# Atarilab/iterative_learning_NMPC

Measured on AMD Instinct MI355X. Metric: MPC solves/sec (horizon-50 centroidal, batch), higher is better.
Workload: dtype f32; 1 GPU; configs[1]: batch=1024/GPU centroidal quadruped NMPC nx=12 nu=12 N=50 fp32, 1 SQP x 6 IPM Riccati sweeps per solve, warm-start shift + solve per step; global_batch=1024, horizon=50, parallelism=dp1 (independent problems; no collective)

## Files before the change

iterative_learning_nmpc_amd/csrc/nmpc_models.hpp:

```cpp
#pragma once
#include "nmpc_tile.hpp"

#pragma clang fp contract(off)

namespace nmpc {

struct ModelParams {
    float dt, mass, ixx, iyy, izz, gz, mu, umax;
    float p_gain, hipx, hipy, lhip, l1, l2, res0, res1;
};

struct DoubleIntegrator {
    static constexpr int ID = 0, NX = 4, NU = 2, NP = 0, NG = 4;

    __device__ static void step(const ModelParams& mp, const float (&x)[NX], const float (&u)[NU],
                                const float*, float (&xn)[NX]) {
        const float dt = mp.dt, h2 = 0.5f * dt * dt;
        xn[0] = x[0] + dt * x[2] + h2 * u[0];
        xn[1] = x[1] + dt * x[3] + h2 * u[1];
        xn[2] = x[2] + dt * u[0];
        xn[3] = x[3] + dt * u[1];
    }
    template <class EA, class EB>
    __device__ static void linearize(const ModelParams& mp, const float (&x)[NX], const float (&u)[NU],
                                     const float* p, float (&xn)[NX], EA&& emitA, EB&& emitB) {
        step(mp, x, u, p, xn);
        const float dt = mp.dt, h2 = 0.5f * dt * dt;
        { float c[NX] = {1.f, 0.f, 0.f, 0.f}; emitA(0, c); }
        { float c[NX] = {0.f, 1.f, 0.f, 0.f}; emitA(1, c); }
        { float c[NX] = {dt, 0.f, 1.f, 0.f}; emitA(2, c); }
        { float c[NX] = {0.f, dt, 0.f, 1.f}; emitA(3, c); }
        { float c[NX] = {h2, 0.f, dt, 0.f}; emitB(0, c); }
        { float c[NX] = {0.f, h2, 0.f, dt}; emitB(1, c); }
    }
    __device__ static float G(const ModelParams&, int j, int c) {
        return (c == (j >> 1)) ? ((j & 1) ? -1.f : 1.f) : 0.f;
    }
    __device__ static float h(const ModelParams& mp, int) { return mp.umax; }
    __device__ static unsigned active_mask(const ModelParams& mp, const float*) {
        return mp.umax > 0.f ? 0xFu : 0u;
    }
    __device__ static void gdot(const ModelParams&, const float (&v)[NU], float (&o)[NG]) {
#pragma clang fp contract(off)
        o[0] = v[0]; o[1] = -v[0]; o[2] = v[1]; o[3] = -v[1];
    }
    static constexpr int N_STATIC_MASKS = 1;
    __host__ __device__ static constexpr unsigned static_mask(int) { return 0x3u; }
    __host__ __device__ static constexpr int static_index(unsigned mask) { return mask == 0x3u ? 0 : -1; }
    __host__ __device__ static constexpr int common_variant(int i) { return i == 0 ? 0 : -1; }
    __host__ __device__ static constexpr unsigned barrier_steps(unsigned) { return 0xFu; }
    __device__ static unsigned input_mask(const ModelParams&, const float*) { return 0x3u; }
};

struct Centroidal {
    static constexpr int ID = 1, NX = 12, NU = 12, NP = 16, NG = 16;

    struct Trig { float cz, sz, cy, sy, cx, sx; };

    __device__ static void rot(const Trig& t, float (&R)[9]) {
        R[0] = t.cz * t.cy; R[1] = t.cz * t.sy * t.sx - t.sz * t.cx; R[2] = t.cz * t.sy * t.cx + t.sz * t.sx;
        R[3] = t.sz * t.cy; R[4] = t.sz * t.sy * t.sx + t.cz * t.cx; R[5] = t.sz * t.sy * t.cx - t.cz * t.sx;
        R[6] = -t.sy;       R[7] = t.cy * t.sx;                       R[8] = t.cy * t.cx;
    }
    __device__ static void tmul(const float (&M)[9], const float (&v)[3], float (&o)[3]) {
        o[0] = M[0] * v[0] + M[3] * v[1] + M[6] * v[2];
        o[1] = M[1] * v[0] + M[4] * v[1] + M[7] * v[2];
        o[2] = M[2] * v[0] + M[5] * v[1] + M[8] * v[2];
    }

    struct Core {
        Trig t; float R[9]; float F[3]; float tau[3]; float w[3]; float vn[3]; float wn[3]; float T[9];
    };
    __device__ static void core(const ModelParams& mp, const float (&x)[NX], const float (&u)[NU],
                                const float* p, Core& k) {
        sincosf(x[3], &k.t.sz, &k.t.cz);
        sincosf(x[4], &k.t.sy, &k.t.cy);
        sincosf(x[5], &k.t.sx, &k.t.cx);
        rot(k.t, k.R);
        k.w[0] = x[11]; k.w[1] = x[10]; k.w[2] = x[9];
        k.F[0] = k.F[1] = k.F[2] = 0.f;
        k.tau[0] = k.tau[1] = k.tau[2] = 0.f;
#pragma unroll
        for (int i = 0; i < 4; ++i) {
            const float c = p[i];
// ... 152 lines not shown
        const int d = c - 3 * f;
        return (d == (jj >> 1)) ? ((jj & 1) ? -1.f : 1.f) : (d == 2 ? -mp.mu : 0.f);
    }
    __device__ static float h(const ModelParams&, int) { return 0.f; }
    __device__ static unsigned active_mask(const ModelParams&, const float* p) {
        unsigned m = 0;
#pragma unroll
        for (int f = 0; f < 4; ++f) m |= (p[f] > 0.5f) ? (0x1111u << f) : 0u;
        return m;
    }
    __device__ static unsigned input_mask(const ModelParams&, const float* p) {
        unsigned m = 0;
#pragma unroll
        for (int f = 0; f < 4; ++f) m |= (p[f] > 0.5f) ? (0x7u << (3 * f)) : 0u;
        return m;
    }
    static constexpr int N_STATIC_MASKS = 16;
    __host__ __device__ static constexpr unsigned static_mask(int i) {
        unsigned m = 0;
        for (int f = 0; f < 4; ++f) m |= ((i >> f) & 1) ? (0x7u << (3 * f)) : 0u;
        return m;
    }
    __host__ __device__ static constexpr int common_variant(int i) { return i == 0 ? 9 : i == 1 ? 6 : i == 2 ? 15 : i == 3 ? 0 : -1; }
    __host__ __device__ static constexpr unsigned barrier_steps(unsigned mask) {
        unsigned m = 0;
        for (int f = 0; f < 4; ++f) m |= ((mask >> (3 * f)) & 1u) << f;
        return m;
    }
    __host__ __device__ static constexpr int static_index(unsigned mask) {
        int i = 0;
        for (int f = 0; f < 4; ++f) i |= ((mask >> (3 * f)) & 1u) << f;
        return static_mask(i) == mask ? i : -1;
    }
    __device__ static void gdot(const ModelParams& mp, const float (&v)[NU], float (&o)[NG]) {
#pragma clang fp contract(off)
#pragma unroll
        for (int f = 0; f < 4; ++f) {
            o[row_of(f, 0)] = __builtin_fmaf(-mp.mu, v[3 * f + 2], v[3 * f]);
            o[row_of(f, 1)] = __builtin_fmaf(-mp.mu, v[3 * f + 2], -v[3 * f]);
            o[row_of(f, 2)] = __builtin_fmaf(-mp.mu, v[3 * f + 2], v[3 * f + 1]);
            o[row_of(f, 3)] = __builtin_fmaf(-mp.mu, v[3 * f + 2], -v[3 * f + 1]);
        }
    }
};

}

#pragma clang fp contract(fast)
```

iterative_learning_nmpc_amd/csrc/nmpc_solve.hip:

```cpp
#include <hip/hip_runtime.h>

#include <type_traits>

#include "../../include/nmpc.h"
#include "nmpc_models.hpp"
#include "nmpc_sweep.hpp"

namespace nmpc {

struct SolveArgs {
    ModelParams mp;
    float W[32];
    float rs_free[16];
    float We[16];
    float reg, reg_e;
    int N, B;
    int max_sqp, n_ipm, line_search, yref_per_stage;
    int it;
    int shift;
    float nlp_tol, mu0, sigma, s_min, gamma, tau_min, rho;
    const float* x0;
    const float* yref;
    const float* yref_e;
    const float* params;
// ... 112 lines not shown
        int o = 0;
        Xs = o;  o += round4(nX);
        Us = o;  o += round4(nU);
        dX = o;  o += round4(nX);
        dU = o;  o += round4(nU);
        dXp = o; o += round4(nX);
        dUp = o; o += round4(nU);
        sv = o;  o += round4(nG);
        lv = o;  o += round4(nG);
        o += 4;
        total = o;
    }
};

template <class M>
struct WsLayout {
    size_t At, Bt, Kt, Ct, q, r, c, act, umk, cost, flag, lean, stride;
    __host__ __device__ explicit WsLayout(int N) {
        size_t o = 0;
        At = o; o += (size_t)N * TileGeom<M>::A_FLOATS;
        Bt = o; o += (size_t)N * TileGeom<M>::B_FLOATS;
        Kt = o; o += (size_t)(N + 1) * TileGeom<M>::K_FLOATS;
        Ct = o; o += (size_t)(N + 1) * TileGeom<M>::C_FLOATS;
        q = o; o += round4((N + 1) * M::NX);
        r = o; o += round4(N * M::NU);
        c = o; o += round4(N * M::NG);
        act = o; o += round4(N);
        umk = o; o += round4(N);
        cost = o; o += round4(N + 1);
        flag = o; o += 4;
        lean = o; o += StageArrays<M>(N, true).total;
        stride = (o + 63) & ~(size_t)63;
    }
};
constexpr int N_LANE_STAGES = 4;
__host__ __device__ constexpr bool qp_linearizes_itself(bool lean, int N) { return lean && N < 64; }

#ifdef NMPC_STAMPS
#define STAMP_DECL unsigned long long st_t0 = __builtin_readcyclecounter(), st_acc[8] = {0, 0, 0, 0, 0, 0, 0, 0}; \
    StageStamps sst = {0, {0, 0, 0, 0, 0, 0, 0, 0}}
#define SST_PASS , sst
#define SST_TILES(i) SST(i)
#define STAMP(i) do { const unsigned long long st_t1 = __builtin_readcyclecounter(); st_acc[i] += st_t1 - st_t0; st_t0 = st_t1; } while (0)
#else
#define STAMP_DECL
#define STAMP(i)
#define SST_PASS
#define SST_TILES(i)
#endif

template <class M, bool LEAN>
struct Lds {
    int arr, qv, rv, gsq, gvt, act, umk, conv, dx0, total;
    __host__ __device__ explicit Lds(int N) {
        const int NS = (N + 1) | 1;
        int o = 0;
        arr = o; o += LEAN ? 0 : StageArrays<M>(N, false).total;
        qv = o;  o += (N + 1) * TS;
        rv = o;  o += N * TS;
        gsq = o; o += N * TS;
        gvt = o; o += N * TS;
        act = o; o += round4(NS);
        umk = o; o += round4(NS);
        conv = o; o += CONV_FLOATS;
        dx0 = o; o += LEAN ? TS : 0;
        total = o;
    }
};

constexpr int LIN_LDS_FLOATS = 64 * 16 + 2 * 64 * 2;
template <class M>
__device__ __forceinline__ void linearize_node(const SolveArgs& a, bool in_range, int b_in, int k_in, float* lds) {
#pragma clang fp contract(off)
    constexpr int NX = M::NX, NU = M::NU, NP = M::NP, NG = M::NG, NY = NX + NU;
    using G = TileGeom<M>;
    float* stage_col = lds;
    float** tile_of0 = reinterpret_cast<float**>(lds + 64 * 16);
    float** tile_of1 = tile_of0 + 64;
    float** tile_of[2] = {tile_of0, tile_of1};
    const int N = a.N;
    const int tid = threadIdx.x;
    const int b = b_in;
    const int k = in_range ? k_in : N;
    const WsLayout<M> wl(N);
    float* ws = a.ws + (size_t)b * wl.stride;
    const bool live = in_range && !(a.it > 0 && reinterpret_cast<const int*>(ws + wl.flag)[0]) && !skipped(a, b);
    const bool stage = live && k < N;
    const int ks = stage ? k : 0;
    const float* Xg = a.X + (size_t)b * (N + 1) * NX;
    const float* Ug = a.U + (size_t)b * N * NU;
    tile_of[0][tid] = stage ? ws + wl.At + (size_t)k * G::A_FLOATS : nullptr;
    tile_of[1][tid] = stage ? ws + wl.Bt + (size_t)k * G::B_FLOATS : nullptr;
    float x[NX];
#pragma unroll
    for (int i = 0; i < NX; ++i) x[i] = Xg[(size_t)shifted_node(live ? k : 0, a.shift, N) * NX + i];
    if (live && k == N) {
// ... 125 lines not shown
}

#pragma clang fp contract(off)
#ifndef NMPC_RES_WAVES
#define NMPC_RES_WAVES 1
#endif
template <class M, bool LEAN, bool BF16B, bool ALLV>
__global__ __launch_bounds__(64) __attribute__((amdgpu_waves_per_eu(LEAN ? 2 : NMPC_RES_WAVES, LEAN ? 2 : NMPC_RES_WAVES)))
void nmpc_qp_kernel(const SolveArgs a) {
    constexpr int NX = M::NX, NU = M::NU, NP = M::NP, NG = M::NG, NY = NX + NU;
    using G = TileGeom<M>;
    extern __shared__ __attribute__((aligned(16))) float smem[];
    const int b = blockIdx.x;
    if (b >= a.B) return;
    if (skipped(a, b)) return;
    const int lane = lane_id();
    const int q4 = lane >> 4, c = lane & 15;
    const int N = a.N;
    const WsLayout<M> wl(N);
    float* ws = a.ws + (size_t)b * wl.stride;
    int* flag = reinterpret_cast<int*>(ws + wl.flag);
    if (a.it > 0 && flag[0]) return;
    const Lds<M, LEAN> L(N);
    const StageArrays<M> SA_(N, LEAN);
    const int NS = SA_.NS;
    float* arr = LEAN ? ws + wl.lean : smem + L.arr;
    float* Xs = arr + SA_.Xs;   float* Us = arr + SA_.Us;
    float* dX = arr + SA_.dX;   float* dU = arr + SA_.dU;
    float* dXp = arr + SA_.dXp; float* dUp = arr + SA_.dUp;
    float* sv = arr + SA_.sv;   float* lv = arr + SA_.lv;
    float* idle_sink = arr + SA_.total - 4;
    float* qv = smem + L.qv;   float* rv = smem + L.rv;
    float* gsq = smem + L.gsq; float* gvt = smem + L.gvt;
    auto phase_sync = [&]() {
        if constexpr (LEAN) __threadfence_block();
        wave_sync();
    };
    unsigned* actm = reinterpret_cast<unsigned*>(smem + L.act);
    unsigned* umask = reinterpret_cast<unsigned*>(smem + L.umk);
    float* conv = smem + L.conv;
#define AT(arr, k, i) (arr)[LEAN ? (k) * TS + (i) : (i) * NS + (k)]
    auto ld_row = [&](const float* arr_, int k, auto& out) {
        constexpr int n = (int)(sizeof(out) / sizeof(float));
        if constexpr (LEAN) {
#pragma unroll
            for (int g = 0; g < (n + 3) / 4; ++g) {
                const f32x4 v = *reinterpret_cast<const f32x4*>(arr_ + k * TS + 4 * g);
#pragma unroll
                for (int r = 0; r < 4; ++r)
                    if (4 * g + r < n) out[4 * g + r] = v[r];
            }
        } else {
#pragma unroll
            for (int i = 0; i < n; ++i) out[i] = AT(arr_, k, i);
        }
    };
    auto st_row = [&](float* arr_, int k, const auto& in) {
        constexpr int n = (int)(sizeof(in) / sizeof(float));
        if constexpr (LEAN) {
#pragma unroll
            for (int g = 0; g < (n + 3) / 4; ++g) {
                f32x4 v;
#pragma unroll
                for (int r = 0; r < 4; ++r) v[r] = (4 * g + r < n) ? in[4 * g + r < n ? 4 * g + r : 0] : 0.0f;
                *reinterpret_cast<f32x4*>(arr_ + k * TS + 4 * g) = v;
            }
        } else {
#pragma unroll
            for (int i = 0; i < n; ++i) AT(arr_, k, i) = in[i];
        }
    };

    float* Xg = a.X + (size_t)b * (N + 1) * NX;
    float* Ug = a.U + (size_t)b * N * NU;
    const float* pg = a.params + (size_t)b * (N + 1) * NP;
    const float* yr = a.yref + (size_t)b * (a.yref_per_stage ? (size_t)N * NY : (size_t)NY);
    const float* yre = a.yref_e + (size_t)b * NX;
    const float* x0 = a.x0 + (size_t)b * NX;
    float* At = ws + wl.At;
    float* Bt = ws + wl.Bt;
    float* Kt = ws + wl.Kt;
    float* Ct = ws + wl.Ct;

    if constexpr (LEAN) {
        if (qp_linearizes_itself(LEAN, N)) {
            static_assert(LIN_LDS_FLOATS <= 4 * TS * 20, "scratch of the fused linearisation");
            linearize_node<M>(a, lane <= N, b, lane, smem + L.qv);
            __threadfence_block();
            wave_sync();
        }
    }
    for (int i = 4 * lane; i < L.conv; i += 256)
        *reinterpret_cast<f32x4*>(smem + i) = zero4();
    if constexpr (LEAN)
        for (int i = 4 * lane; i < SA_.total; i += 256) *reinterpret_cast<f32x4*>(arr + i) = zero4();
    phase_sync();
    constexpr int PRE = 13;
    auto fetch = [&](const float* src, int total, int base, float (&v)[PRE]) {
#pragma unroll
        for (int u = 0; u < PRE; ++u) {
            const int e = base + 64 * u + lane;
            v[u] = src[e < total ? e : 0];
// ... 44 lines not shown
        fetch(ws + wl.c, n_c, base, vc);
        drain(n_x, base, vx, put_x);
        drain(n_x, base, vq, put_q);
        drain(n_u, base, vu, put_u);
        drain(n_u, base, vr, put_r);
        drain(n_c, base, vc, put_c);
    }
    float* dx0s = smem + L.dx0;
    if constexpr (LEAN) {
        if (lane < NX) dx0s[lane] = x0[lane] - Xg[lane];
    }
    float cost_l = 0.0f, mu_l = 0.0f;
    int nact_l = 0;
    for (int k = lane; k <= N; k += 64) {
        cost_l += ws[wl.cost + k];
        if (k < N) {
            const unsigned am = reinterpret_cast<const unsigned*>(ws + wl.act)[k];
            actm[k] = am;
            const unsigned um = reinterpret_cast<const unsigned*>(ws + wl.umk)[k];
            const unsigned um_prev = reinterpret_cast<const unsigned*>(ws + wl.umk)[k > 0 ? k - 1 : 0];
            const unsigned wider = (k > 0 && (M::barrier_steps(um_prev) & ~M::barrier_steps(um)) != 0u) ? 1u : 0u;
            umask[k] = um | ((unsigned)(M::static_index(um) + 1) << 16) | (wider << 24);
            nact_l += __popc(am);
            mu_l += a.mu0 * (float)__popc(am);
        }
    }
    const int ic = index_of(c);
    const bool c_is_x = ic >= 0 && ic < NX, c_is_u = ic >= 0 && ic < NU;
    const float wq_c = c_is_x ? a.W[c_is_x ? ic : 0] + a.reg : 0.0f;
    const float wr_c = c_is_u ? a.W[NX + (c_is_u ? ic : 0)] + a.reg : 0.0f;
    const float we_c = c_is_x ? a.We[c_is_x ? ic : 0] + a.reg_e : 0.0f;
    SweepLane sl;
    sl.init(conv, lane, HS, a.rs_free);
    f32x4 Qc, Rc, Gc;
    bool qm[4], rm[4];
#pragma unroll
    for (int r = 0; r < 4; ++r) {
        const int row = 4 * q4 + r, ir = index_of(row);
        const bool r_is_x = ir >= 0 && ir < NX, r_is_u = ir >= 0 && ir < NU;
        Qc[r] = (row == c && r_is_x) ? wq_c : 0.0f;
        Rc[r] = (row == c && r_is_u) ? wr_c : 0.0f;
        qm[r] = (c == HS && r_is_x) || (row == HS && c_is_x);
        rm[r] = (c == HS && r_is_u);
        Gc[r] = (row < NG && c_is_u) ? M::G(a.mp, row < NG ? row : 0, c_is_u ? ic : 0) : 0.0f;
    }
    const bool is_hx_col = (c == HS);
    phase_sync();

    int status = NMPC_STATUS_MAXITER;
    bool finished = false;
    STAMP_DECL;
    float cost = 0.0f, stepn = 0.0f, alpha = 1.0f;
    const bool rows_in_regs = LEAN && N < 64;
    const int kx_s = lane <= N ? lane : 0, ku_s = lane < N ? lane : 0;
    float xr[LEAN ? NX : 1], ur[LEAN ? NU : 1];
    {
        cost = wave_sum(cost_l);
        const int n_act = (int)(wave_sum((float)nact_l) + 0.5f);
        STAMP(0);
        const bool use_ipm = (a.n_ipm > 0) && (n_act > 0);
        const int n_sweeps = use_ipm ? a.n_ipm : 1;
        bool qp_ok = true;
        float mu_sum = wave_sum(mu_l);
        const bool one_stage_per_lane = N <= 64;
        auto blend = [&](float ap) {
            batched<10>(SA_.nX, lane, [&](int i) { const float d = dX[i]; return __builtin_fmaf(ap, dXp[i] - d, d); },
                        [&](int i, float v) { dX[i] = v; });
            batched<10>(SA_.nU, lane, [&](int i) { const float d = dU[i]; return __builtin_fmaf(ap, dUp[i] - d, d); },
                        [&](int i, float v) { dU[i] = v; });
        };
        for (int ii = 0; ii < n_sweeps; ++ii) {
            float tau = 0.0f;
            if (use_ipm) {
                tau = fmaxf(a.sigma * mu_sum / (float)n_act, a.tau_min);
                if (ii == 0 || !one_stage_per_lane)
                for (int k = lane; k < N; k += 64) {
                    const unsigned am = actm[k];
                    float uk[NU], gk[NG], sk[NG], lk[NG];
                    ld_row(Us, k, uk);
                    ld_row(sv, k, sk);
                    ld_row(lv, k, lk);
                    M::gdot(a.mp, uk, gk);
#pragma unroll
                    for (int j = 0; j < NG; ++j) {
                        const bool on = (am >> j) & 1u;
                        const float s = sk[j], l = lk[j], cj = gk[j] - M::h(a.mp, j);
                        const float is = fast_rcp(s);
                        const float D = l * is;
                        const float rs = __builtin_amdgcn_rsqf(D);
                        gsq[k * TS + j] = on ? D * rs : 0.0f;
                        gvt[k * TS + j] = on ? __builtin_fmaf(D, cj, __builtin_fmaf(tau, is, l)) * rs : 0.0f;
                    }
                }
                phase_sync();
            }
            STAMP(1);
            f32x4 P;
            {
                const float qc = c_is_x ? qv[N * TS + c] : 0.0f;
#pragma unroll
                for (int r = 0; r < 4; ++r) {
                    const int row = 4 * q4 + r, ir = index_of(row);
                    const bool r_is_x = ir >= 0 && ir < NX;
                    float v = 0.0f;
                    if (row == c && r_is_x) v = we_c;
                    if (c == HS && r_is_x) v = qv[N * TS + row];
                    if (row == HS && c_is_x) v = qc;
                    P[r] = v;
                }
            }
            auto sweep = [&](auto ipm_tag) {
                constexpr bool IPM = decltype(ipm_tag)::value;
                struct NextCost {
                    f32x4 Gs, Vt, Tb, Qn, Sn, Rn;
                    const float *qrow, *rrow, *sqrow, *vtrow;
                    const float* qcol;
                    const bool *qm, *rm;
                    f32x4 Qc, Rc, Gc;
                    bool hx_col;
                    f32x4 q4v, r4v, sq4, vt4;
                    float qcv;
                    __device__ __forceinline__ void fetch() {
                        q4v = *reinterpret_cast<const f32x4*>(qrow);
                        r4v = *reinterpret_cast<const f32x4*>(rrow);
                        qcv = *qcol;
                        if constexpr (IPM) {
                            sq4 = *reinterpret_cast<const f32x4*>(sqrow);
                            vt4 = *reinterpret_cast<const f32x4*>(vtrow);
                        }
                    }
                    __device__ __forceinline__ void build() {
                        Rn = Rc;
#pragma unroll
                        for (int r = 0; r < 4; ++r) {
                            Qn[r] = Qc[r] + (qm[r] ? (hx_col ? q4v[r] : qcv) : 0.0f);
                            Sn[r] = rm[r] ? r4v[r] : 0.0f;
                        }
                        if constexpr (IPM) {
#pragma unroll
                            for (int r = 0; r < 4; ++r) {
                                Gs[r] = Gc[r] * sq4[r];
                                Vt[r] = hx_col ? vt4[r] : Gs[r];
                            }
                            Tb = zero4();
                        }
                    }
                    __device__ __forceinline__ void mfma(int i) {
                        if constexpr (IPM && !BF16B) Tb = __builtin_amdgcn_mfma_f32_16x16x4f32(Gs[i], Vt[i], Tb, 0, 0, 0);
                        if constexpr (IPM && BF16B) { if (i == 0) Tb = xty_bf16(Gs, Vt); }
                    }
                    __device__ __forceinline__ void finish() {
                        if constexpr (IPM) {
#pragma unroll
                            for (int r = 0; r < 4; ++r) {
                                Rn[r] += hx_col ? 0.0f : Tb[r];
                                Sn[r] += hx_col ? Tb[r] : 0.0f;
                            }
                        }
                    }
                };
                auto next_cost = [&](int kk) {
                    NextCost nc;
                    nc.qrow = qv + kk * TS + 4 * q4; nc.rrow = rv + kk * TS + 4 * q4;
                    nc.sqrow = gsq + kk * TS + 4 * q4; nc.vtrow = gvt + kk * TS + 4 * q4;
                    nc.qcol = qv + kk * TS + c;
                    nc.qm = qm; nc.rm = rm;
                    nc.Qc = Qc; nc.Rc = Rc; nc.Gc = Gc; nc.hx_col = is_hx_col;
                    return nc;
                };
                ImageLane<M> il;
                il.init(lane);
                RowStoreLane ks, cs;
                ks.init(lane, G::KQ, G::K_FLOATS, N - 1, N);
                cs.init(lane, G::CQ, G::C_FLOATS, N - 1, N);
                f32x4 A0 = il.fix_A(il.load_A(At + (size_t)(N - 1) * G::A_FLOATS), lane);
                f32x4 B0 = il.fix_B(il.load_B(Bt + (size_t)(N - 1) * G::B_FLOATS), lane);
                f32x4 T0 = il.fix_Bt(il.load_Bt(Bt + (size_t)(N - 1) * G::B_FLOATS), lane);
                f32x4 Qt, St, Rt;
                {
                    NextCost nc = next_cost(N - 1);
                    nc.fetch();
                    nc.build();
#pragma unroll
                    for (int i = 0; i < 4; ++i) nc.mfma(i);
                    nc.finish();
                    Qt = nc.Qn; St = nc.Sn; Rt = nc.Rn;
                }
                unsigned cm = umask[N - 1];
                int lane_zero = 0;
                asm volatile("" : "+v"(lane_zero));
                for (int k = N - 1; k >= 0; --k) {
#ifdef NMPC_STAMPS
                    sst.t0 = __builtin_readcyclecounter();
#endif
                    const int kn = (k > 0) ? k - 1 : 0;
#ifdef QP_T_ONEIMG
                    const int ki = (a.B < 0) ? kn : 0;
#else
                    const int ki = kn;
#endif
                    const f32x4 A1 = il.load_A(At + (size_t)ki * G::A_FLOATS);
                    const f32x4 B1 = il.load_B(Bt + (size_t)ki * G::B_FLOATS);
                    const f32x4 T1 = il.load_Bt(Bt + (size_t)ki * G::B_FLOATS);
                    const unsigned cm_next = umask[kn + lane_zero];
                    f32x4 Kk, Acl;
                    NextCost sh = next_cost(kn);
                    auto run = [&](auto mask_tag) {
                        constexpr unsigned MK = decltype(mask_tag)::value;
                        constexpr unsigned STEPS = (IPM && !BF16B && MK != DYNAMIC_MASK) ? M::barrier_steps(MK) : 0xFu;
                        return backward_stage<NU, MK, true, ALLV, STEPS, LEAN ? 0 : 2>(P, A0, B0, T0, Qt, St, Rt, conv, sl, lane,
                                                                        cm & 0xFFFFu, Kk, Acl, sh SST_PASS);
                    };
                    bool ok = true;
#define NMPC_VARIANT(I)                                                                                   \
    case I:                                                                                               \
        if constexpr (I < M::N_STATIC_MASKS)                                                              \
            ok = run(std::integral_constant<unsigned, M::static_mask(I < M::N_STATIC_MASKS ? I : 0)>{}); \
        else ok = run(std::integral_constant<unsigned, DYNAMIC_MASK>{});                                  \
        break;
#define NMPC_COMMON(J) (M::common_variant(J) >= 0 && vi == M::common_variant(J))
#define NMPC_RUN_COMMON(J) run(std::integral_constant<unsigned, M::static_mask(M::common_variant(J) >= 0 ? M::common_variant(J) : 0)>{})
                    constexpr int WIDEST = M::static_index((NU < 32) ? ((1u << NU) - 1u) : 0xFFFFFFFFu);
                    const int vi = ((cm >> 24) & 1u) ? WIDEST : (int)((cm >> 16) & 0x1Fu) - 1;
                    if constexpr (!ALLV) {
                        if (NMPC_COMMON(0)) ok = NMPC_RUN_COMMON(0);
                        else if (NMPC_COMMON(1)) ok = NMPC_RUN_COMMON(1);
                        else if (NMPC_COMMON(2)) ok = NMPC_RUN_COMMON(2);
                        else if (NMPC_COMMON(3)) ok = NMPC_RUN_COMMON(3);
                        else ok = run(std::integral_constant<unsigned, DYNAMIC_MASK>{});
                    } else {
                        switch (vi) {
                            NMPC_VARIANT(0) NMPC_VARIANT(1) NMPC_VARIANT(2) NMPC_VARIANT(3)
                            NMPC_VARIANT(4) NMPC_VARIANT(5) NMPC_VARIANT(6) NMPC_VARIANT(7)
                            NMPC_VARIANT(8) NMPC_VARIANT(9) NMPC_VARIANT(10) NMPC_VARIANT(11)
                            NMPC_VARIANT(12) NMPC_VARIANT(13) NMPC_VARIANT(14) NMPC_VARIANT(15)
                            default: ok = run(std::integral_constant<unsigned, DYNAMIC_MASK>{});
                        }
                    }
#undef NMPC_VARIANT
#undef NMPC_COMMON
#undef NMPC_RUN_COMMON
                    qp_ok = ok && qp_ok;
#ifdef QP_T_NOSTORE
                    if (a.B < 0)
#endif
                    {
                    ks.store(Kt, Kk);
                    cs.store(Ct, Acl);
                    }
                    A0 = il.fix_A(A1, lane);
                    B0 = il.fix_B(B1, lane);
                    T0 = il.fix_Bt(T1, lane);
                    Qt = sh.Qn; St = sh.Sn; Rt = sh.Rn;
                    cm = __builtin_amdgcn_readfirstlane(cm_next);
                    SST_TILES(5);
                }
            };
            if (use_ipm) sweep(std::true_type{}); else sweep(std::false_type{});
            __threadfence_block();
            wave_sync();
            STAMP(2);
            float* oX = use_ipm ? dXp : dX;
            float* oU = use_ipm ? dUp : dU;
            float vs[NX];
            if constexpr (LEAN) {
#pragma unroll
                for (int i = 0; i < NX; ++i) vs[i] = dx0s[i];
                if (lane < NX) AT(oX, 0, lane) = dx0s[lane];
            } else {
#pragma unroll
                for (int i = 0; i < NX; ++i) vs[i] = x0[i] - AT(Xs, 0, i);
                if (lane < NX) AT(oX, 0, lane) = x0[lane] - AT(Xs, 0, lane);
            }
            constexpr int FWD_PF = 4, RQ4 = slot_of(NX - 1) / 4 + 1;
            const bool is_x = lane < NX, is_u = (lane >= 16 && lane < 16 + NU);
            unsigned rowoff = 4u * (unsigned)((is_x ? wl.Ct : wl.Kt) + (is_x ? lane : is_u ? lane - 16 : 0) * TS);
            const unsigned rowstep = 4u * (is_x ? G::C_FLOATS : G::K_FLOATS);
            float* dst = is_x ? &AT(oX, 1, lane) : is_u ? &AT(oU, 0, lane - 16) : idle_sink;
            const int dstep = (is_x || is_u) ? (LEAN ? TS : 1) : 0;
            auto load_row = [&](unsigned off, f32x4 (&row)[RQ4]) {
                row[0] = *reinterpret_cast<const f32x4*>(reinterpret_cast<const char*>(ws) + (size_t)off);
#pragma unroll
                for (int g = 1; g < RQ4; ++g) {
                    const f32x3u v = *reinterpret_cast<const f32x3u*>(reinterpret_cast<const char*>(ws) + (size_t)off + 16 * g);
                    row[g] = f32x4{v[0], v[1], v[2], 0.0f};
                }
            };
            f32x4 ring[FWD_PF][RQ4];
// ... 55 lines not shown
                    const bool on = (am >> j) & 1u;
                    rp = on ? fmaxf(rp, -ds[j] * is) : rp;
                    rd = on ? fmaxf(rd, -dl[j] * __builtin_amdgcn_rcpf(l[j])) : rd;
                }
                const float rpm = wave_max(rp), rdm = wave_max(rd);
                const float ap = rpm > a.gamma ? a.gamma / rpm : 1.0f;
                const float ad = rdm > a.gamma ? a.gamma / rdm : 1.0f;
                float m_l = 0.0f;
#pragma unroll
                for (int j = 0; j < NG; ++j) {
                    const bool on = (am >> j) & 1u;
                    s[j] = on ? __builtin_fmaf(ap, ds[j], s[j]) : s[j];
                    l[j] = on ? __builtin_fmaf(ad, dl[j], l[j]) : l[j];
                    m_l = on ? __builtin_fmaf(s[j], l[j], m_l) : m_l;
                }
                if (live) { st_row(sv, k, s); st_row(lv, k, l); }
                mu_sum = wave_sum(m_l);
                if constexpr (LEAN) {
#pragma unroll
                    for (int i = 0; i < NX; ++i) dxo[i] = __builtin_fmaf(ap, dxn[i] - dxo[i], dxo[i]);
#pragma unroll
                    for (int i = 0; i < NU; ++i) duo[i] = __builtin_fmaf(ap, du[i] - duo[i], duo[i]);
                    if (lane <= N) st_row(dX, kx, dxo);
                    if (live) st_row(dU, k, duo);
                    if (N == 64 && lane < NX) {
                        const float d = AT(dX, 64, lane);
                        AT(dX, 64, lane) = __builtin_fmaf(ap, AT(dXp, 64, lane) - d, d);
                    }
                } else {
                    blend(ap);
                }
                if (ii + 1 < n_sweeps && live) {
                    const float tau_n = fmaxf(a.sigma * mu_sum / (float)n_act, a.tau_min);
                    float sq[NG], vt[NG];
#pragma unroll
                    for (int j = 0; j < NG; ++j) {
                        const bool on = (am >> j) & 1u;
                        const float is = fast_rcp(s[j]);
                        const float D = l[j] * is;
                        const float rs = __builtin_amdgcn_rsqf(D);
                        sq[j] = on ? D * rs : 0.0f;
                        vt[j] = on ? __builtin_fmaf(D, cc[j], __builtin_fmaf(tau_n, is, l[j])) * rs : 0.0f;
                    }
#pragma unroll
                    for (int j = 0; j < NG; ++j) { gsq[k * TS + j] = sq[j]; gvt[k * TS + j] = vt[j]; }
                }
                phase_sync();
            } else if (use_ipm) {
                float ap_l = 1.0f, ad_l = 1.0f;
                auto step_dir = [&](int k, int j, const float (&g)[NG], const float (&cc)[NG], float& s, float& l, float& dsj, float& dlj) {
                    s = AT(sv, k, j); l = AT(lv, k, j);
                    const float is = fast_rcp(s);
                    dsj = -(g[j] + cc[j]) - s;
                    dlj = __builtin_fmaf(-(l * is), dsj, __builtin_fmaf(tau, is, -l));
                };
                for (int k = lane; k < N; k += 64) {
                    float du[NU], g[NG], uk[NU], cc[NG];
#pragma unroll
                    for (int i = 0; i < NU; ++i) { du[i] = AT(dUp, k, i); uk[i] = AT(Us, k, i); }
                    M::gdot(a.mp, du, g);
                    M::gdot(a.mp, uk, cc);
#pragma unroll
                    for (int j = 0; j < NG; ++j) cc[j] -= M::h(a.mp, j);
                    const unsigned am = actm[k];
#pragma unroll
                    for (int j = 0; j < NG; ++j) {
                        float s, l, dsj, dlj;
                        step_dir(k, j, g, cc, s, l, dsj, dlj);
                        const bool on = (am >> j) & 1u;
                        if (on && dsj < 0.0f) ap_l = fminf(ap_l, -a.gamma * s / dsj);
                        if (on && dlj < 0.0f) ad_l = fminf(ad_l, -a.gamma * l / dlj);
                    }
                }
                const float ap = wave_min(ap_l), ad = wave_min(ad_l);
                float m_l = 0.0f;
                for (int k = lane; k < N; k += 64) {
                    float du[NU], g[NG], uk[NU], cc[NG];
#pragma unroll
// ... 156 lines not shown
```

Before: 2.223 million solves/s.

## Precompute per-foot barrier Hessian blocks instead of MFMA in Riccati sweep

```diff
diff --git a/iterative_learning_nmpc_amd/csrc/nmpc_models.hpp b/iterative_learning_nmpc_amd/csrc/nmpc_models.hpp
--- a/iterative_learning_nmpc_amd/csrc/nmpc_models.hpp
+++ b/iterative_learning_nmpc_amd/csrc/nmpc_models.hpp
@@ -50,6 +50,7 @@
     __host__ __device__ static constexpr int common_variant(int i) { return i == 0 ? 0 : -1; }
     __host__ __device__ static constexpr unsigned barrier_steps(unsigned) { return 0xFu; }
     __device__ static unsigned input_mask(const ModelParams&, const float*) { return 0x3u; }
+    static constexpr bool HAS_BARRIER_BLOCKS = false;
 };
 
 struct Centroidal {
@@ -268,6 +269,33 @@
         for (int f = 0; f < 4; ++f) i |= ((mask >> (3 * f)) & 1u) << f;
         return static_mask(i) == mask ? i : -1;
     }
+    static constexpr bool HAS_BARRIER_BLOCKS = true;
+    static constexpr int FOOT_FLOATS = 8, BLOCK_FLOATS = 4 * FOOT_FLOATS;
+    __host__ __device__ static constexpr int block_entry(int a, int b) {
+        return a == b ? 3 + a : (a + b == 2) ? 6 : (a + b == 3) ? 7 : -1;
+    }
+    __device__ static void barrier_foot(const ModelParams& mp, int f, const float (&sq)[4], const float (&vt)[4],
+                                        const float (&r)[3], const float (&rdiag)[3], float (&o)[FOOT_FLOATS]) {
+#pragma clang fp contract(off)
+        float gs[4][3];
+#pragma unroll
+        for (int jj = 0; jj < 4; ++jj)
+#pragma unroll
+            for (int d = 0; d < 3; ++d) gs[jj][d] = G(mp, row_of(f, jj), 3 * f + d) * sq[jj];
+        auto chain = [&](int a, int b) {
+            float acc = 0.0f;
+#pragma unroll
+            for (int jj = 0; jj < 4; ++jj) acc = __builtin_fmaf(gs[jj][a], b < 3 ? gs[jj][b < 3 ? b : 0] : vt[jj], acc);
+            return acc;
+        };
+#pragma unroll
+        for (int d = 0; d < 3; ++d) {
+            o[d] = r[d] + chain(d, 3);
+            o[3 + d] = rdiag[d] + chain(d, d);
+        }
+        o[6] = 0.0f + chain(0, 2);
+        o[7] = 0.0f + chain(1, 2);
+    }
     __device__ static void gdot(const ModelParams& mp, const float (&v)[NU], float (&o)[NG]) {
 #pragma clang fp contract(off)
 #pragma unroll
diff --git a/iterative_learning_nmpc_amd/csrc/nmpc_solve.hip b/iterative_learning_nmpc_amd/csrc/nmpc_solve.hip
--- a/iterative_learning_nmpc_amd/csrc/nmpc_solve.hip
+++ b/iterative_learning_nmpc_amd/csrc/nmpc_solve.hip
@@ -168,6 +168,16 @@
         lean = o; o += StageArrays<M>(N, true).total;
         stride = (o + 63) & ~(size_t)63;
     }
+};
+template <class M, bool = M::HAS_BARRIER_BLOCKS>
+struct BarrierRecord {
+    static constexpr int FOOT_FLOATS = 0, BLOCK_FLOATS = 0;
+    __host__ __device__ static constexpr int entry(int, int) { return -1; }
+};
+template <class M>
+struct BarrierRecord<M, true> {
+    static constexpr int FOOT_FLOATS = M::FOOT_FLOATS, BLOCK_FLOATS = M::BLOCK_FLOATS;
+    __host__ __device__ static constexpr int entry(int a, int b) { return M::block_entry(a, b); }
 };
 constexpr int N_LANE_STAGES = 4;
 __host__ __device__ constexpr bool qp_linearizes_itself(bool lean, int N) { return lean && N < 64; }
@@ -389,6 +399,9 @@
     float* idle_sink = arr + SA_.total - 4;
     float* qv = smem + L.qv;   float* rv = smem + L.rv;
     float* gsq = smem + L.gsq; float* gvt = smem + L.gvt;
+    constexpr bool BLK = M::HAS_BARRIER_BLOCKS && !BF16B;
+    float* brec = gsq;
+    static_assert(!BLK || 2 * TS == 32, "the record takes the place of gsq and gvt");
     auto phase_sync = [&]() {
         if constexpr (LEAN) __threadfence_block();
         wave_sync();
@@ -425,6 +438,52 @@
         } else {
 #pragma unroll
             for (int i = 0; i < n; ++i) AT(arr_, k, i) = in[i];
+        }
+    };
+
+    auto rdiag_quad = [&](int f) { return conv + 3 * CTILE + (1 + f) * LDC + TS; };
+    auto put_barrier = [&](int k, unsigned am, const float (&sk)[NG], const float (&lk)[NG], const float (&ck)[NG], float tau_k) {
+        auto coef = [&](int j, float& sq, float& vt) {
+            const bool on = (am >> j) & 1u;
+            const float is = fast_rcp(sk[j]);
+            const float D = lk[j] * is;
+            const float rs = __builtin_amdgcn_rsqf(D);
+            sq = on ? D * rs : 0.0f;
+            vt = on ? __builtin_fmaf(D, ck[j], __builtin_fmaf(tau_k, is, lk[j])) * rs : 0.0f;
+        };
+        if constexpr (BLK) {
+            static_assert(M::BLOCK_FLOATS == 2 * TS, "the record takes the place of gsq and gvt");
+            float rk[NU];
+            if constexpr (!LEAN) {
+#pragma unroll
+                for (int i = 0; i < NU; ++i) rk[i] = rv[k * TS + slot_of(i)];
+            }
+#pragma unroll
+            for (int f = 0; f < 4; ++f) {
+                float sq[4], vt[4], o[M::FOOT_FLOATS];
+                if constexpr (LEAN) {
+                    __builtin_amdgcn_sched_barrier(0);
+#pragma unroll
+                    for (int d = 0; d < 3; ++d) rk[3 * f + d] = rv[k * TS + slot_of(3 * f + d)];
+                }
+#pragma unroll
+                for (int jj = 0; jj < 4; ++jj) coef(M::row_of(f, jj), sq[jj], vt[jj]);
+                const float r3[3] = {rk[3 * f], rk[3 * f + 1], rk[3 * f + 2]};
+                const f32x4 rdq = *reinterpret_cast<const f32x4*>(rdiag_quad(f));
+                const float rd3[3] = {rdq[0], rdq[1], rdq[2]};
+                M::barrier_foot(a.mp, f, sq, vt, r3, rd3, o);
+                f32x4* dst = reinterpret_cast<f32x4*>(brec + k * M::BLOCK_FLOATS + f * M::FOOT_FLOATS);
+                dst[0] = f32x4{o[0], o[1], o[2], o[3]};
+                dst[1] = f32x4{o[4], o[5], o[6], o[7]};
+            }
+        } else {
+#pragma unroll
+            for (int j = 0; j < NG; ++j) {
+                float sq, vt;
+                coef(j, sq, vt);
+                gsq[k * TS + j] = sq;
+                gvt[k * TS + j] = vt;
+            }
         }
     };
 
@@ -535,19 +594,17 @@
     const float we_c = c_is_x ? a.We[c_is_x ? ic : 0] + a.reg_e : 0.0f;
     SweepLane sl;
     sl.init(conv, lane, HS, a.rs_free);
-    f32x4 Qc, Rc, Gc;
-    bool qm[4], rm[4];
+    f32x4 Gc;
 #pragma unroll
     for (int r = 0; r < 4; ++r) {
-        const int row = 4 * q4 + r, ir = index_of(row);
-        const bool r_is_x = ir >= 0 && ir < NX, r_is_u = ir >= 0 && ir < NU;
-        Qc[r] = (row == c && r_is_x) ? wq_c : 0.0f;
-        Rc[r] = (row == c && r_is_u) ? wr_c : 0.0f;
-        qm[r] = (c == HS && r_is_x) || (row == HS && c_is_x);
-        rm[r] = (c == HS && r_is_u);
+        const int row = 4 * q4 + r;
         Gc[r] = (row < NG && c_is_u) ? M::G(a.mp, row < NG ? row : 0, c_is_u ? ic : 0) : 0.0f;
     }
-    const bool is_hx_col = (c == HS);
+    if constexpr (BLK) {
+        static_assert(LDC >= TS + 4 && NU <= 3 * (TS - 1), "padding rows of the identity tile hold the zero quad and R + reg per foot");
+        wave_sync();
+        if (q4 == 0 && c_is_u) rdiag_quad(ic / 3)[ic % 3] = wr_c;
+    }
     phase_sync();
 
     int status = NMPC_STATUS_MAXITER;
@@ -585,15 +642,8 @@
                     ld_row(lv, k, lk);
                     M::gdot(a.mp, uk, gk);
 #pragma unroll
-                    for (int j = 0; j < NG; ++j) {
-                        const bool on = (am >> j) & 1u;
-                        const float s = sk[j], l = lk[j], cj = gk[j] - M::h(a.mp, j);
-                        const float is = fast_rcp(s);
-                        const float D = l * is;
-                        const float rs = __builtin_amdgcn_rsqf(D);
-                        gsq[k * TS + j] = on ? D * rs : 0.0f;
-                        gvt[k * TS + j] = on ? __builtin_fmaf(D, cj, __builtin_fmaf(tau, is, l)) * rs : 0.0f;
-                    }
+                    for (int j = 0; j < NG; ++j) gk[j] -= M::h(a.mp, j);
+                    put_barrier(k, am, sk, lk, gk, tau);
                 }
                 phase_sync();
             }
@@ -614,46 +664,63 @@
             }
             auto sweep = [&](auto ipm_tag) {
                 constexpr bool IPM = decltype(ipm_tag)::value;
+                constexpr bool REC = IPM && BLK;
                 struct NextCost {
-                    f32x4 Gs, Vt, Tb, Qn, Sn, Rn;
-                    const float *qrow, *rrow, *sqrow, *vtrow;
+                    f32x4 Qn, Sn, Rn;
+                    const float* qrow;
                     const float* qcol;
-                    const bool *qm, *rm;
-                    f32x4 Qc, Rc, Gc;
+                    const float* qmf;
+                    f32x4 Qc, q4v;
+                    float qcv;
+                    const float* brow[3];
+                    const float* srow;
+                    f32x4 rec_r, rec_s;
+                    const float *rrow, *sqrow, *vtrow;
+                    const bool* rm;
+                    f32x4 Rc, Gc, r4v, sq4, vt4, Gs, Vt, Tb;
                     bool hx_col;
-                    f32x4 q4v, r4v, sq4, vt4;
-                    float qcv;
                     __device__ __forceinline__ void fetch() {
                         q4v = *reinterpret_cast<const f32x4*>(qrow);
-                        r4v = *reinterpret_cast<const f32x4*>(rrow);
                         qcv = *qcol;
-                        if constexpr (IPM) {
-                            sq4 = *reinterpret_cast<const f32x4*>(sqrow);
-                            vt4 = *reinterpret_cast<const f32x4*>(vtrow);
+                        if constexpr (REC) {
+#pragma unroll
+                            for (int r = 0; r < 3; ++r) rec_r[r] = *brow[r];
+                            rec_s = *reinterpret_cast<const f32x4*>(srow);
+                        } else {
+                            r4v = *reinterpret_cast<const f32x4*>(rrow);
+                            if constexpr (IPM) {
+                                sq4 = *reinterpret_cast<const f32x4*>(sqrow);
+                                vt4 = *reinterpret_cast<const f32x4*>(vtrow);
+                            }
                         }
                     }
                     __device__ __forceinline__ void build() {
-                        Rn = Rc;
-#pragma unroll
-                        for (int r = 0; r < 4; ++r) {
-                            Qn[r] = Qc[r] + (qm[r] ? (hx_col ? q4v[r] : qcv) : 0.0f);
-                            Sn[r] = rm[r] ? r4v[r] : 0.0f;
+                        static_assert(HS == 3, "the q border relies on the homogeneous slot being register 3 of quad 0");
+#pragma unroll
+                        for (int r = 0; r < 4; ++r) Qn[r] = __builtin_fmaf(qmf[r], r < 3 ? q4v[r] : qcv, Qc[r]);
+                        if constexpr (REC) {
+                            Rn = f32x4{rec_r[0], rec_r[1], rec_r[2], 0.0f};
+                            Sn = f32x4{rec_s[0], rec_s[1], rec_s[2], 0.0f};
+                        } else {
+                            Rn = Rc;
+#pragma unroll
+                            for (int r = 0; r < 4; ++r) Sn[r] = rm[r] ? r4v[r] : 0.0f;
+                            if constexpr (IPM) {
+#pragma unroll
+                                for (int r = 0; r < 4; ++r) {
+                                    Gs[r] = Gc[r] * sq4[r];
+                                    Vt[r] = hx_col ? vt4[r] : Gs[r];
+                                }
+                                Tb = zero4();
+                            }
                         }
-                        if constexpr (IPM) {
-#pragma unroll
-                            for (int r = 0; r < 4; ++r) {
-                                Gs[r] = Gc[r] * sq4[r];
-                                Vt[r] = hx_col ? vt4[r] : Gs[r];
-                            }
-                            Tb = zero4();
-                        }
                     }
                     __device__ __forceinline__ void mfma(int i) {
-                        if constexpr (IPM && !BF16B) Tb = __builtin_amdgcn_mfma_f32_16x16x4f32(Gs[i], Vt[i], Tb, 0, 0, 0);
+                        if constexpr (IPM && !BF16B && !REC) Tb = __builtin_amdgcn_mfma_f32_16x16x4f32(Gs[i], Vt[i], Tb, 0, 0, 0);
                         if constexpr (IPM && BF16B) { if (i == 0) Tb = xty_bf16(Gs, Vt); }
                     }
                     __device__ __forceinline__ void finish() {
-                        if constexpr (IPM) {
+                        if constexpr (IPM && !REC) {
 #pragma unroll
                             for (int r = 0; r < 4; ++r) {
                                 Rn[r] += hx_col ? 0.0f : Tb[r];
@@ -662,13 +729,52 @@
                         }
                     }
                 };
+                int lane_zero = 0;
+                asm volatile("" : "+v"(lane_zero));
+                const int q4s = (lane + lane_zero) >> 4, cs_ = (lane + lane_zero) & 15;
+                float qmf[4];
+                bool rm[4];
+                const bool is_hx_col = (cs_ == HS);
+                f32x4 Qc, Rc;
+#pragma unroll
+                for (int r = 0; r < 4; ++r) {
+                    const int ir = index_of(4 * q4s + r), icl = index_of(cs_);
+                    Qc[r] = (4 * q4s + r == cs_ && ir >= 0 && ir < NX) ? wq_c : 0.0f;
+                    Rc[r] = (4 * q4s + r == cs_ && ir >= 0 && ir < NU) ? wr_c : 0.0f;
+                    rm[r] = (cs_ == HS && ir >= 0 && ir < NU);
+                    qmf[r] = ((cs_ == HS && ir >= 0 && ir < NX) || (4 * q4s + r == HS && icl >= 0 && icl < NX)) ? 1.0f : 0.0f;
+                }
+                using BR = BarrierRecord<M>;
+                int b_off[3] = {0, 0, 0}, b_step[3] = {0, 0, 0}, s_off = 0, s_step = 0;
+                if constexpr (IPM && BLK) {
+                    static_assert(LDC >= TS + 4, "zero quad behind a column of the identity tile");
+                    const int zero_quad = L.conv + 3 * CTILE + TS;
+                    const int d = cs_ & 3;
+                    const bool in_block = (cs_ >> 2) == q4s && d < 3;
+#pragma unroll
+                    for (int r = 0; r < 3; ++r) {
+                        const int e = BR::entry(r, d < 3 ? d : 0);
+                        const bool used = in_block && e >= 0;
+                        b_off[r] = used ? L.gsq + q4s * BR::FOOT_FLOATS + e : zero_quad;
+                        b_step[r] = used ? BR::BLOCK_FLOATS : 0;
+                    }
+                    s_off = (cs_ == HS) ? L.gsq + q4s * BR::FOOT_FLOATS : zero_quad;
+                    s_step = (cs_ == HS) ? BR::BLOCK_FLOATS : 0;
+                }
                 auto next_cost = [&](int kk) {
                     NextCost nc;
-                    nc.qrow = qv + kk * TS + 4 * q4; nc.rrow = rv + kk * TS + 4 * q4;
-                    nc.sqrow = gsq + kk * TS + 4 * q4; nc.vtrow = gvt + kk * TS + 4 * q4;
+                    nc.qrow = qv + kk * TS + 4 * q4;
                     nc.qcol = qv + kk * TS + c;
-                    nc.qm = qm; nc.rm = rm;
-                    nc.Qc = Qc; nc.Rc = Rc; nc.Gc = Gc; nc.hx_col = is_hx_col;
+                    nc.qmf = qmf; nc.Qc = Qc;
+                    if constexpr (REC) {
+#pragma unroll
+                        for (int r = 0; r < 3; ++r) nc.brow[r] = smem + b_off[r] + kk * b_step[r];
+                        nc.srow = smem + s_off + kk * s_step;
+                    } else {
+                        nc.rrow = rv + kk * TS + 4 * q4;
+                        nc.sqrow = gsq + kk * TS + 4 * q4; nc.vtrow = gvt + kk * TS + 4 * q4;
+                        nc.rm = rm; nc.Rc = Rc; nc.Gc = Gc; nc.hx_col = is_hx_col;
+                    }
                     return nc;
                 };
                 ImageLane<M> il;
@@ -690,8 +796,6 @@
                     Qt = nc.Qn; St = nc.Sn; Rt = nc.Rn;
                 }
                 unsigned cm = umask[N - 1];
-                int lane_zero = 0;
-                asm volatile("" : "+v"(lane_zero));
                 for (int k = N - 1; k >= 0; --k) {
 #ifdef NMPC_STAMPS
                     sst.t0 = __builtin_readcyclecounter();
@@ -878,18 +982,7 @@
                 }
                 if (ii + 1 < n_sweeps && live) {
                     const float tau_n = fmaxf(a.sigma * mu_sum / (float)n_act, a.tau_min);
-                    float sq[NG], vt[NG];
-#pragma unroll
-                    for (int j = 0; j < NG; ++j) {
-                        const bool on = (am >> j) & 1u;
-                        const float is = fast_rcp(s[j]);
-                        const float D = l[j] * is;
-                        const float rs = __builtin_amdgcn_rsqf(D);
-                        sq[j] = on ? D * rs : 0.0f;
-                        vt[j] = on ? __builtin_fmaf(D, cc[j], __builtin_fmaf(tau_n, is, l[j])) * rs : 0.0f;
-                    }
-#pragma unroll
-                    for (int j = 0; j < NG; ++j) { gsq[k * TS + j] = sq[j]; gvt[k * TS + j] = vt[j]; }
+                    put_barrier(k, am, s, l, cc, tau_n);
                 }
                 phase_sync();
             } else if (use_ipm) {
```

Result: faster. 2.274 million solves/s (median of 6 runs) (+2.3%).

## Dispatch backward Riccati sweep per run of equal mask variants, not per stage

Applied to the files above, without the earlier changes.

```diff
diff --git a/iterative_learning_nmpc_amd/csrc/nmpc_solve.hip b/iterative_learning_nmpc_amd/csrc/nmpc_solve.hip
--- a/iterative_learning_nmpc_amd/csrc/nmpc_solve.hip
+++ b/iterative_learning_nmpc_amd/csrc/nmpc_solve.hip
@@ -187,7 +187,7 @@
 
 template <class M, bool LEAN>
 struct Lds {
-    int arr, qv, rv, gsq, gvt, act, umk, conv, dx0, total;
+    int arr, qv, rv, gsq, gvt, act, umk, runs, conv, dx0, total;
     __host__ __device__ explicit Lds(int N) {
         const int NS = (N + 1) | 1;
         int o = 0;
@@ -198,6 +198,7 @@
         gvt = o; o += N * TS;
         act = o; o += round4(NS);
         umk = o; o += round4(NS);
+        runs = o; o += LEAN ? 0 : round4(N + 1);
         conv = o; o += CONV_FLOATS;
         dx0 = o; o += LEAN ? TS : 0;
         total = o;
@@ -549,6 +550,42 @@
     }
     const bool is_hx_col = (c == HS);
     phase_sync();
+    constexpr int WIDEST = M::static_index((NU < 32) ? ((1u << NU) - 1u) : 0xFFFFFFFFu);
+    constexpr unsigned KEY_DYNAMIC = ALLV ? 16u : 4u;
+    auto run_key = [&](unsigned w) -> unsigned {
+        const int vi = ((w >> 24) & 1u) ? WIDEST : (int)((w >> 16) & 0x1Fu) - 1;
+        if constexpr (ALLV) {
+            return (vi >= 0 && vi < 16 && vi < M::N_STATIC_MASKS) ? (unsigned)vi : KEY_DYNAMIC;
+        } else {
+            unsigned key = KEY_DYNAMIC;
+#pragma unroll
+            for (int j = 3; j >= 0; --j)
+                if (M::common_variant(j) >= 0 && vi == M::common_variant(j)) key = (unsigned)j;
+            return key;
+        }
+    };
+    unsigned* runs = reinterpret_cast<unsigned*>(smem + L.runs);
+    if constexpr (!LEAN) {
+        int n_runs = 0;
+        for (int base = ((N - 1) >> 6) << 6; base >= 0; base -= 64) {
+            const int k = base + lane;
+            const bool valid = k < N;
+            const unsigned w = umask[valid ? k : N - 1], w_above = umask[k + 1 < N ? k + 1 : N - 1];
+            const unsigned key = run_key(w);
+            const bool first = valid && (k == N - 1 || key != run_key(w_above) || (((w | w_above) >> 24) & 1u) != 0u);
+            const unsigned long long m = __ballot(first);
+            const unsigned long long above = (lane < 63) ? (m >> (lane + 1)) : 0ull;
+            if (first) runs[n_runs + __popcll(above)] = (key << 18) | (unsigned)(k + 1);
+            n_runs += __popcll(m);
+        }
+        if (lane == 0) runs[n_runs] = 0u;
+        wave_sync();
+        for (int i = lane; i < n_runs; i += 64) {
+            const unsigned w = runs[i], w_next = runs[i + 1];
+            runs[i] = w | (((w & 0x1FFu) - (w_next & 0x1FFu)) << 9);
+        }
+        wave_sync();
+    }
 
     int status = NMPC_STATUS_MAXITER;
     bool finished = false;
@@ -689,74 +726,150 @@
                     nc.finish();
                     Qt = nc.Qn; St = nc.Sn; Rt = nc.Rn;
                 }
-                unsigned cm = umask[N - 1];
                 int lane_zero = 0;
                 asm volatile("" : "+v"(lane_zero));
-                for (int k = N - 1; k >= 0; --k) {
+                if constexpr (LEAN) {
+                    unsigned cm = umask[N - 1];
+                    for (int k = N - 1; k >= 0; --k) {
+    #ifdef NMPC_STAMPS
+                        sst.t0 = __builtin_readcyclecounter();
+    #endif
+                        const int kn = (k > 0) ? k - 1 : 0;
+    #ifdef QP_T_ONEIMG
+                        const int ki = (a.B < 0) ? kn : 0;
+    #else
+                        const int ki = kn;
+    #endif
+                        const f32x4 A1 = il.load_A(At + (size_t)ki * G::A_FLOATS);
+                        const f32x4 B1 = il.load_B(Bt + (size_t)ki * G::B_FLOATS);
+                        const f32x4 T1 = il.load_Bt(Bt + (size_t)ki * G::B_FLOATS);
+                        const unsigned cm_next = umask[kn + lane_zero];
+                        f32x4 Kk, Acl;
+                        NextCost sh = next_cost(kn);
+                        auto run = [&](auto mask_tag) {
+                            constexpr unsigned MK = decltype(mask_tag)::value;
+                            constexpr unsigned STEPS = (IPM && !BF16B && MK != DYNAMIC_MASK) ? M::barrier_steps(MK) : 0xFu;
+                            return backward_stage<NU, MK, true, ALLV, STEPS, LEAN ? 0 : 2>(P, A0, B0, T0, Qt, St, Rt, conv, sl, lane,
+                                                                            cm & 0xFFFFu, Kk, Acl, sh SST_PASS);
+                        };
+                        bool ok = true;
+    #define NMPC_VARIANT(I)                                                                                   \
+        case I:                                                                                               \
+            if constexpr (I < M::N_STATIC_MASKS)                                                              \
+                ok = run(std::integral_constant<unsigned, M::static_mask(I < M::N_STATIC_MASKS ? I : 0)>{}); \
+            else ok = run(std::integral_constant<unsigned, DYNAMIC_MASK>{});                                  \
+            break;
+    #define NMPC_COMMON(J) (M::common_variant(J) >= 0 && vi == M::common_variant(J))
+    #define NMPC_RUN_COMMON(J) run(std::integral_constant<unsigned, M::static_mask(M::common_variant(J) >= 0 ? M::common_variant(J) : 0)>{})
+                        const int vi = ((cm >> 24) & 1u) ? WIDEST : (int)((cm >> 16) & 0x1Fu) - 1;
+                        if constexpr (!ALLV) {
+                            if (NMPC_COMMON(0)) ok = NMPC_RUN_COMMON(0);
+                            else if (NMPC_COMMON(1)) ok = NMPC_RUN_COMMON(1);
+                            else if (NMPC_COMMON(2)) ok = NMPC_RUN_COMMON(2);
+                            else if (NMPC_COMMON(3)) ok = NMPC_RUN_COMMON(3);
+                            else ok = run(std::integral_constant<unsigned, DYNAMIC_MASK>{});
+                        } else {
+                            switch (vi) {
+                                NMPC_VARIANT(0) NMPC_VARIANT(1) NMPC_VARIANT(2) NMPC_VARIANT(3)
+                                NMPC_VARIANT(4) NMPC_VARIANT(5) NMPC_VARIANT(6) NMPC_VARIANT(7)
+                                NMPC_VARIANT(8) NMPC_VARIANT(9) NMPC_VARIANT(10) NMPC_VARIANT(11)
+                                NMPC_VARIANT(12) NMPC_VARIANT(13) NMPC_VARIANT(14) NMPC_VARIANT(15)
+                                default: ok = run(std::integral_constant<unsigned, DYNAMIC_MASK>{});
+                            }
+                        }
+    #undef NMPC_VARIANT
+    #undef NMPC_COMMON
+    #undef NMPC_RUN_COMMON
+                        qp_ok = ok && qp_ok;
+    #ifdef QP_T_NOSTORE
+                        if (a.B < 0)
+    #endif
+                        {
+                        ks.store(Kt, Kk);
+                        cs.store(Ct, Acl);
+                        }
+                        A0 = il.fix_A(A1, lane);
+                        B0 = il.fix_B(B1, lane);
+                        T0 = il.fix_Bt(T1, lane);
+                        Qt = sh.Qn; St = sh.Sn; Rt = sh.Rn;
+                        cm = __builtin_amdgcn_readfirstlane(cm_next);
+                        SST_TILES(5);
+                    }
+                } else {
+                    auto run_stages = [&](auto mask_tag, int top, int len) {
+                        constexpr unsigned MK = decltype(mask_tag)::value;
+                        constexpr bool DYN = (MK == DYNAMIC_MASK);
+                        constexpr unsigned STEPS = (IPM && !BF16B && !DYN) ? M::barrier_steps(MK) : 0xFu;
+                        unsigned cm = 0u;
+                        if constexpr (DYN) cm = __builtin_amdgcn_readfirstlane(umask[top - 1]);
+                        for (int k = top - 1; k >= top - len; --k) {
 #ifdef NMPC_STAMPS
-                    sst.t0 = __builtin_readcyclecounter();
+                            sst.t0 = __builtin_readcyclecounter();
 #endif
-                    const int kn = (k > 0) ? k - 1 : 0;
+                            const int kn = (k > 0) ? k - 1 : 0;
 #ifdef QP_T_ONEIMG
-                    const int ki = (a.B < 0) ? kn : 0;
+                            const int ki = (a.B < 0) ? kn : 0;
 #else
-                    const int ki = kn;
+                            const int ki = kn;
 #endif
-                    const f32x4 A1 = il.load_A(At + (size_t)ki * G::A_FLOATS);
-                    const f32x4 B1 = il.load_B(Bt + (size_t)ki * G::B_FLOATS);
-                    const f32x4 T1 = il.load_Bt(Bt + (size_t)ki * G::B_FLOATS);
-                    const unsigned cm_next = umask[kn + lane_zero];
-                    f32x4 Kk, Acl;
-                    NextCost sh = next_cost(kn);
-                    auto run = [&](auto mask_tag) {
-                        constexpr unsigned MK = decltype(mask_tag)::value;
-                        constexpr unsigned STEPS = (IPM && !BF16B && MK != DYNAMIC_MASK) ? M::barrier_steps(MK) : 0xFu;
-                        return backward_stage<NU, MK, true, ALLV, STEPS, LEAN ? 0 : 2>(P, A0, B0, T0, Qt, St, Rt, conv, sl, lane,
-                                                                        cm & 0xFFFFu, Kk, Acl, sh SST_PASS);
+                            const f32x4 A1 = il.load_A(At + (size_t)ki * G::A_FLOATS);
+                            const f32x4 B1 = il.load_B(Bt + (size_t)ki * G::B_FLOATS);
+                            const f32x4 T1 = il.load_Bt(Bt + (size_t)ki * G::B_FLOATS);
+                            unsigned cm_next = 0u;
+                            if constexpr (DYN) cm_next = umask[kn + lane_zero];
+                            f32x4 Kk, Acl;
+                            NextCost sh = next_cost(kn);
+                            const bool ok = backward_stage<NU, MK, true, ALLV, STEPS, LEAN ? 0 : 2>(P, A0, B0, T0, Qt, St, Rt, conv, sl, lane,
+                                                                                                 cm & 0xFFFFu, Kk, Acl, sh SST_PASS);
+                            qp_ok = ok && qp_ok;
+#ifdef QP_T_NOSTORE
+                            if (a.B < 0)
+#endif
+                            {
+                            ks.store(Kt, Kk);
+                            cs.store(Ct, Acl);
+                            }
+                            A0 = il.fix_A(A1, lane);
+                            B0 = il.fix_B(B1, lane);
+                            T0 = il.fix_Bt(T1, lane);
+                            Qt = sh.Qn; St = sh.Sn; Rt = sh.Rn;
+                            if constexpr (DYN) cm = __builtin_amdgcn_readfirstlane(cm_next);
+                            SST_TILES(5);
+                        }
                     };
-                    bool ok = true;
-#define NMPC_VARIANT(I)                                                                                   \
-    case I:                                                                                               \
-        if constexpr (I < M::N_STATIC_MASKS)                                                              \
-            ok = run(std::integral_constant<unsigned, M::static_mask(I < M::N_STATIC_MASKS ? I : 0)>{}); \
-        else ok = run(std::integral_constant<unsigned, DYNAMIC_MASK>{});                                  \
-        break;
-#define NMPC_COMMON(J) (M::common_variant(J) >= 0 && vi == M::common_variant(J))
-#define NMPC_RUN_COMMON(J) run(std::integral_constant<unsigned, M::static_mask(M::common_variant(J) >= 0 ? M::common_variant(J) : 0)>{})
-                    constexpr int WIDEST = M::static_index((NU < 32) ? ((1u << NU) - 1u) : 0xFFFFFFFFu);
-                    const int vi = ((cm >> 24) & 1u) ? WIDEST : (int)((cm >> 16) & 0x1Fu) - 1;
-                    if constexpr (!ALLV) {
-                        if (NMPC_COMMON(0)) ok = NMPC_RUN_COMMON(0);
-                        else if (NMPC_COMMON(1)) ok = NMPC_RUN_COMMON(1);
-                        else if (NMPC_COMMON(2)) ok = NMPC_RUN_COMMON(2);
-                        else if (NMPC_COMMON(3)) ok = NMPC_RUN_COMMON(3);
-                        else ok = run(std::integral_constant<unsigned, DYNAMIC_MASK>{});
-                    } else {
-                        switch (vi) {
-                            NMPC_VARIANT(0) NMPC_VARIANT(1) NMPC_VARIANT(2) NMPC_VARIANT(3)
-                            NMPC_VARIANT(4) NMPC_VARIANT(5) NMPC_VARIANT(6) NMPC_VARIANT(7)
-                            NMPC_VARIANT(8) NMPC_VARIANT(9) NMPC_VARIANT(10) NMPC_VARIANT(11)
-                            NMPC_VARIANT(12) NMPC_VARIANT(13) NMPC_VARIANT(14) NMPC_VARIANT(15)
-                            default: ok = run(std::integral_constant<unsigned, DYNAMIC_MASK>{});
+#define NMPC_VARIANT(I)                                                                                                 \
+        case I:                                                                                                             \
+            if constexpr (I < M::N_STATIC_MASKS)                                                                            \
+                run_stages(std::integral_constant<unsigned, M::static_mask(I < M::N_STATIC_MASKS ? I : 0)>{}, top, len);    \
+            else run_stages(std::integral_constant<unsigned, DYNAMIC_MASK>{}, top, len);                                    \
+            break;
+#define NMPC_COMMON(J) (M::common_variant(J) >= 0 && key == J##u)
+#define NMPC_RUN_COMMON(J) run_stages(std::integral_constant<unsigned, M::static_mask(M::common_variant(J) >= 0 ? M::common_variant(J) : 0)>{}, top, len)
+                    unsigned rw = __builtin_amdgcn_readfirstlane(runs[0]);
+                    for (int r = 1; (rw & 0x1FFu) != 0u; ++r) {
+                        const unsigned rw_next = runs[r + lane_zero];
+                        const int top = (int)(rw & 0x1FFu), len = (int)((rw >> 9) & 0x1FFu);
+                        const unsigned key = rw >> 18;
+                        if constexpr (!ALLV) {
+                            if (NMPC_COMMON(0)) NMPC_RUN_COMMON(0);
+                            else if (NMPC_COMMON(1)) NMPC_RUN_COMMON(1);
+                            else if (NMPC_COMMON(2)) NMPC_RUN_COMMON(2);
+                            else if (NMPC_COMMON(3)) NMPC_RUN_COMMON(3);
+                            else run_stages(std::integral_constant<unsigned, DYNAMIC_MASK>{}, top, len);
+                        } else {
+                            switch (key) {
+                                NMPC_VARIANT(0) NMPC_VARIANT(1) NMPC_VARIANT(2) NMPC_VARIANT(3)
+                                NMPC_VARIANT(4) NMPC_VARIANT(5) NMPC_VARIANT(6) NMPC_VARIANT(7)
+                                NMPC_VARIANT(8) NMPC_VARIANT(9) NMPC_VARIANT(10) NMPC_VARIANT(11)
+                                NMPC_VARIANT(12) NMPC_VARIANT(13) NMPC_VARIANT(14) NMPC_VARIANT(15)
+                                default: run_stages(std::integral_constant<unsigned, DYNAMIC_MASK>{}, top, len);
+                            }
                         }
+                        rw = __builtin_amdgcn_readfirstlane(rw_next);
                     }
 #undef NMPC_VARIANT
 #undef NMPC_COMMON
 #undef NMPC_RUN_COMMON
-                    qp_ok = ok && qp_ok;
-#ifdef QP_T_NOSTORE
-                    if (a.B < 0)
-#endif
-                    {
-                    ks.store(Kt, Kk);
-                    cs.store(Ct, Acl);
-                    }
-                    A0 = il.fix_A(A1, lane);
-                    B0 = il.fix_B(B1, lane);
-                    T0 = il.fix_Bt(T1, lane);
-                    Qt = sh.Qn; St = sh.Sn; Rt = sh.Rn;
-                    cm = __builtin_amdgcn_readfirstlane(cm_next);
-                    SST_TILES(5);
                 }
             };
             if (use_ipm) sweep(std::true_type{}); else sweep(std::false_type{});
```

After: 2.230 million solves/s before, 2.417 million solves/s after, median of 6. +8.4%, better.
